# freshman97/LinTransUNet

Measured on AMD Instinct MI355X. Metric: 128^3 CT patches/sec (fwd+bwd), higher is better.
Workload: dtype bf16; 1 GPU; MaskTransUnet train step (fwd + 5-level loss + bwd), 128^3 single-channel patches, 2 per GPU, dropout 0.3, random-init weights; global_batch=2, parallelism=dp1, side_stream_concurrent=True, allreduce=none (1 rank)

## Files before the change

### lintransunet_amd/csrc/sdgrad_ring.hip

```cpp
#include "gemm_desc.h"
#include "lds_dma.h"

struct SdEnt { int c, dh, dw, dd, tap; };
template <int SD>
__host__ __device__ constexpr SdEnt sd_entry(int e) {
  int idx = 0, cls = 0;
  for (int ph = 0; ph < 2; ++ph)
    for (int pw = 0; pw < 2; ++pw)
      for (int pd = 0; pd < SD; ++pd) {
        const int nh = ph ? 2 : 1, nw = pw ? 2 : 1, nd = SD == 2 ? (pd ? 2 : 1) : 3;
        for (int i = 0; i < nh; ++i)
          for (int j = 0; j < nw; ++j)
            for (int k = 0; k < nd; ++k) {
              if (idx == e) {
                const int oh = ph ? (i == 0 ? 1 : 0) : 0, th = ph ? (i == 0 ? 0 : 2) : 1;
                const int ow = pw ? (j == 0 ? 1 : 0) : 0, tw = pw ? (j == 0 ? 0 : 2) : 1;
                const int od = SD == 2 ? (pd ? (k == 0 ? 1 : 0) : 0) : 1 - k;
                const int td = SD == 2 ? (pd ? (k == 0 ? 0 : 2) : 1) : k;
                return SdEnt{cls, oh, ow, od, (th * 3 + tw) * 3 + td};
              }
              ++idx;
            }
        ++cls;
      }
  return SdEnt{0, 0, 0, 0, -1};
}

struct SdgradArgs {
  const uint16_t* g;
  const uint16_t* w;
  uint16_t* dx;
  int B, Ho, Wo, Do, Co;
  int Hl, Wl, Dl, N;
  int tap[28];
};

template <int SD>
__global__ void __launch_bounds__(256) sdgrad_ring_bf16_kernel(const SdgradArgs a) {
  constexpr int NC = SD == 2 ? 8 : 4;
  constexpr int HH = 5, HW = 9, HD = SD == 2 ? 9 : 10;
  constexpr int NR = HH * HW * HD, HP = ((NR + 15) / 16 + 3) / 4;
  constexpr int HBUF = 4 * HP * 1024;
  constexpr int WSTAGE = 20 * 1024;
  constexpr int RING = 2 * HBUF;
  constexpr int OD0 = SD == 2 ? 0 : 1;
  extern __shared__ __attribute__((aligned(1024))) char smem[];
  const int tid = threadIdx.x, lane = tid & 63, wave = tid >> 6;
  const int li = lane & 31, lh = lane >> 5;
  const int nbh = (a.Ho + 3) / 4, nbw = (a.Wo + 7) / 8, nbd = (a.Do + 7) / 8;
  const Brick bk = split_brick(blockIdx.x, nbh, nbw, nbd);
  const int b = bk.b, h0 = bk.bh * 4, w0 = bk.bw * 8, d0 = bk.bd * 8;
  const int n_blk = blockIdx.y * 32;
  const int nchunk = a.Co / 32;
  const int total = nchunk * 3;
  const uint32_t lds0 = lds_addr(smem);
  const uint16_t* zsrc = reinterpret_cast<const uint16_t*>(ltu_zero_line) + (lane & 3) * 8;

  const int prow = lane >> 2;
  const uint16_t* hsrc[HP];
#pragma unroll
  for (int s = 0; s < HP; ++s) {
    const int hv = (wave * HP + s) * 16 + prow;
    const int hd = hv % HD, hw = (hv / HD) % HW, hh = hv / (HD * HW);
    const int h = h0 + hh, w = w0 + hw, d = d0 - OD0 + hd;
    const int lc = (lane & 3) ^ (hw & 3);
    const bool in = hv < NR && (unsigned)h < (unsigned)a.Ho && (unsigned)w < (unsigned)a.Wo && (unsigned)d < (unsigned)a.Do;
    hsrc[s] = in ? a.g + ((((long long)b * a.Ho + h) * a.Wo + w) * a.Do + d) * a.Co + lc * 8 : zsrc;
  }
  const uint16_t* wsrc[3][5];
#pragma unroll
  for (int s = 0; s < 5; ++s) {
    const int row = (wave * 5 + s) * 16 + prow;
    const int t = row >> 5, n = n_blk + (row & 31);
    const int wchunk = (lane & 3) ^ ((lane >> 4) & 3);
#pragma unroll
    for (int st = 0; st < 3; ++st) {
      const int tap = t < 9 ? a.tap[st * 9 + t] : 27;
      wsrc[st][s] = (tap < 27 && n < a.N) ? a.w + ((long long)n * 27 + tap) * a.Co + wchunk * 8 : zsrc;
    }
  }
  asm volatile("s_waitcnt vmcnt(0)" ::: "memory");

  auto issue_halo = [&](int chunk) {
    const uint32_t hb = lds0 + (chunk & 1) * HBUF + wave * HP * 1024;
#pragma unroll
    for (int s = 0; s < HP; ++s) glds16(hsrc[s] + chunk * 32, hb + s * 1024);
  };
  auto issue_w = [&](int chunk, auto ST) {
    constexpr int st = decltype(ST)::value;
    const uint32_t wb = lds0 + RING + st * WSTAGE + wave * 5 * 1024;
#pragma unroll
    for (int s = 0; s < 5; ++s) glds16(wsrc[st][s] + chunk * 32, wb + s * 1024);
  };

  const int hwl = li >> 3;
  int baseA[2][2][2];
#pragma unroll
  for (int i = 0; i < 2; ++i) {
    const int hv0 = ((wave * HW) + (i * 4 + hwl)) * HD + (li & 7);
#pragma unroll
    for (int ks = 0; ks < 2; ++ks)
#pragma unroll
      for (int dw = 0; dw < 2; ++dw) baseA[i][ks][dw] = hv0 * 64 + (((ks * 2 + lh) ^ ((hwl + dw) & 3)) << 4);
  }
  int baseW[2];
#pragma unroll
  for (int ks = 0; ks < 2; ++ks) baseW[ks] = RING + li * 64 + (((ks * 2 + lh) ^ ((li >> 2) & 3)) << 4);

  f32x16 acc[NC][2];
#pragma unroll
  for (int c = 0; c < NC; ++c)
#pragma unroll
    for (int i = 0; i < 2; ++i)
#pragma unroll
      for (int r = 0; r < 16; ++r) acc[c][i][r] = 0.f;

  issue_halo(0);
  issue_w(0, std::integral_constant<int, 0>{});
  issue_w(0, std::integral_constant<int, 1>{});
  for (int chunk = 0; chunk < nchunk; ++chunk) {
    const int hoff = (chunk & 1) * HBUF;
    int bA[2][2][2];
#pragma unroll
    for (int i = 0; i < 2; ++i)
#pragma unroll
      for (int ks = 0; ks < 2; ++ks)
#pragma unroll
        for (int dw = 0; dw < 2; ++dw) bA[i][ks][dw] = baseA[i][ks][dw] + hoff;
    static_for<0, 3>([&](auto ST) {
      constexpr int st = decltype(ST)::value;
      const int g = chunk * 3 + st;
      if (g + 1 < total) {
        if (st != 0 && chunk + 1 < nchunk) ring_sync<5 + HP>(); else ring_sync<5>();
      } else {
        ring_sync<0>();
      }
      if (g + 2 < total) {
        if constexpr (st == 0) issue_w(chunk, std::integral_constant<int, 2>{});
        else issue_w(chunk + 1, std::integral_constant<int, st - 1>{});
      }
      if (st == 0 && chunk + 1 < nchunk) issue_halo(chunk + 1);
      constexpr int NE = 9;
      auto load_frags = [&](auto TT, bf16x8 (&af)[2][2], bf16x8 (&wf)[2]) {
        constexpr int t = decltype(TT)::value;
        constexpr SdEnt en = sd_entry<SD>(st * 9 + t);
        constexpr int immA = ((en.dh * HW + en.dw) * HD + en.dd + OD0) * 64;
        constexpr int immW = st * WSTAGE + t * 2048;
#pragma unroll
        for (int i = 0; i < 2; ++i)
#pragma unroll
          for (int ks = 0; ks < 2; ++ks) af[i][ks] = *reinterpret_cast<const bf16x8*>(smem + bA[i][ks][en.dw] + immA);
#pragma unroll
        for (int ks = 0; ks < 2; ++ks) wf[ks] = *reinterpret_cast<const bf16x8*>(smem + baseW[ks] + immW);
      };
      auto mma = [&](auto TT, const bf16x8 (&af)[2][2], const bf16x8 (&wf)[2]) {
        constexpr int c = sd_entry<SD>(st * 9 + decltype(TT)::value).c;
#pragma unroll
        for (int ks = 0; ks < 2; ++ks)
#pragma unroll
          for (int i = 0; i < 2; ++i) acc[c][i] = __builtin_amdgcn_mfma_f32_32x32x16_bf16(wf[ks], af[i][ks], acc[c][i], 0, 0, 0);
      };
      bf16x8 afA[2][2], wfA[2], afB[2][2], wfB[2];
      load_frags(std::integral_constant<int, 0>{}, afA, wfA);
      static_for<0, (NE + 1) / 2>([&](auto TP) {
        constexpr int t = decltype(TP)::value * 2;
        if constexpr (t + 1 < NE) load_frags(std::integral_constant<int, t + 1>{}, afB, wfB);
        __builtin_amdgcn_sched_barrier(0);
        mma(std::integral_constant<int, t>{}, afA, wfA);
        __builtin_amdgcn_sched_barrier(0);
        if constexpr (t + 2 < NE) load_frags(std::integral_constant<int, t + 2>{}, afA, wfA);
        __builtin_amdgcn_sched_barrier(0);
        if constexpr (t + 1 < NE) mma(std::integral_constant<int, t + 1>{}, afB, wfB);
        __builtin_amdgcn_sched_barrier(0);
      });
    });
  }

  __syncthreads();
#pragma unroll
  for (int c = 0; c < NC; ++c)
#pragma unroll
    for (int i = 0; i < 2; ++i) {
      const int vox = wave * 64 + i * 32 + li;
      char* row = smem + (c * 256 + vox) * 64;
#pragma unroll
      for (int rr = 0; rr < 4; ++rr) {
        uint2 pk;
        pk.x = pack_bf16x2(acc[c][i][4 * rr + 0], acc[c][i][4 * rr + 1]);
        pk.y = pack_bf16x2(acc[c][i][4 * rr + 2], acc[c][i][4 * rr + 3]);
        *reinterpret_cast<uint2*>(row + ((rr ^ ((vox >> 1) & 3)) << 4) + lh * 8) = pk;
      }
    }
  __syncthreads();
  const int part = tid & 3;
  const bool pok = n_blk + part * 8 < a.N;
  long long vbase[4];
  int qq[4];
#pragma unroll
  for (int k = 0; k < 4; ++k) {
    const int ml = (tid >> 2) + 64 * k;
    const int qh = h0 + (ml >> 6), qw = w0 + ((ml >> 3) & 7), qd = d0 + (ml & 7);
    const bool ok = pok && qh < a.Ho && qw < a.Wo && qd < a.Do;
    vbase[k] = ((((long long)b * a.Hl + 2 * qh) * a.Wl + 2 * qw) * a.Dl + SD * qd) * a.N + n_blk + part * 8;
    qq[k] = ok ? (qh << 20) | (qw << 10) | qd : -1;
  }
#pragma unroll
  for (int c = 0; c < NC; ++c) {
    const int ph = SD == 2 ? c >> 2 : c >> 1, pw = SD == 2 ? (c >> 1) & 1 : c & 1, pd = SD == 2 ? c & 1 : 0;
    const long long coff = ((long long)(ph * a.Wl + pw) * a.Dl + pd) * a.N;
#pragma unroll
    for (int k = 0; k < 4; ++k) {
      const int ml = (tid >> 2) + 64 * k;
      const uint4 v = *reinterpret_cast<const uint4*>(smem + (c * 256 + ml) * 64 + ((part ^ ((ml >> 1) & 3)) << 4));
      const int qh = qq[k] >> 20, qw = (qq[k] >> 10) & 1023, qd = qq[k] & 1023;
      if (qq[k] >= 0 && 2 * qh + ph < a.Hl && 2 * qw + pw < a.Wl && SD * qd + pd < a.Dl)
        *reinterpret_cast<uint4*>(a.dx + vbase[k] + coff) = v;
    }
  }
}

template <int SD>
static int launch_sdgrad(const SdgradArgs& a0, hipStream_t st) {
  SdgradArgs a = a0;
  for (int e = 0; e < 27; ++e) a.tap[e] = sd_entry<SD>(e).tap;
  a.tap[27] = 27;
  constexpr int HD = SD == 2 ? 9 : 10;
  constexpr int HP = ((5 * 9 * HD + 15) / 16 + 3) / 4;
  constexpr int opnd = 2 * 4 * HP * 1024 + 3 * 20 * 1024, epi = (SD == 2 ? 8 : 4) * 256 * 64;
  constexpr int smem_bytes = opnd > epi ? opnd : epi;
  static LtuDevOnce attr_once;
  if (attr_once.first())
    ltu_dyn_lds(&sdgrad_ring_bf16_kernel<SD>, smem_bytes);
  const long long rb = (long long)a.B * ((a.Ho + 3) / 4) * ((a.Wo + 7) / 8) * ((a.Do + 7) / 8);
  if (rb >= (1LL << 31)) return 1;
  hipLaunchKernelGGL(sdgrad_ring_bf16_kernel<SD>, dim3((unsigned)rb, (a.N + 31) / 32), dim3(256), smem_bytes, st, a);
  return ltu_check_launch();
}

int launch_sdgrad_ring_bf16(const void* grad, const void* wd, void* dx, int B, int Hl, int Wl, int Dl, int N, int Co, int sd, hipStream_t st) {
  if (Co % 32 || Co > 512 || N % 8 || (sd != 1 && sd != 2)) return 1;
  SdgradArgs a;
  a.g = (const uint16_t*)grad; a.w = (const uint16_t*)wd; a.dx = (uint16_t*)dx;
  a.B = B; a.Hl = Hl; a.Wl = Wl; a.Dl = Dl; a.N = N; a.Co = Co;
  a.Ho = (Hl - 1) / 2 + 1; a.Wo = (Wl - 1) / 2 + 1; a.Do = (Dl - 1) / sd + 1;
  if (a.Ho < 1 || a.Wo < 1 || a.Do < 1 || a.Ho >= 1024 || a.Wo >= 1024 || a.Do >= 1024) return 1;
  if ((long long)N * 27 * Co >= (1LL << 31)) return 1;
  return sd == 2 ? launch_sdgrad<2>(a, st) : launch_sdgrad<1>(a, st);
}
```

### lintransunet_amd/csrc/upconv_ring.hip

```cpp
#include "gemm_desc.h"
#include "lds_dma.h"

#define UR_HROWS 640
#define UR_HBUF (UR_HROWS * 64)
#define UR_RING (2 * UR_HBUF)
#define UR_WSTAGE 16384
#define UR_SMEM (UR_RING + 4 * UR_WSTAGE)

__host__ __device__ constexpr int ur_off(int p, int a) { return p == 0 ? (a == 0 ? -1 : 0) : (a == 0 ? 0 : 1); }

struct UpRingArgs {
  const uint16_t* x;
  const uint16_t* w;
  const float* bias;
  uint16_t* y;
  int B, H, W, D, Ci, Co;
};

__global__ void __launch_bounds__(256) upconv_ring_bf16_kernel(const UpRingArgs a) {
  extern __shared__ __attribute__((aligned(1024))) char smem[];
  const int tid = threadIdx.x, lane = tid & 63, wave = tid >> 6;
  const int li = lane & 31, lh = lane >> 5;
  const int nbh = (a.H + 3) / 4, nbw = (a.W + 7) / 8, nbd = (a.D + 7) / 8;
  const Brick bk = split_brick(blockIdx.x, nbh, nbw, nbd);
  const int b = bk.b, h0 = bk.bh * 4, w0 = bk.bw * 8, d0 = bk.bd * 8;
  const int n_blk = blockIdx.y * 32;
  const int nchunk = a.Ci / 32;
  const int total = nchunk * 8;
  const uint32_t lds0 = lds_addr(smem);

  const int prow = lane >> 2;
  const uint16_t* hsrc[10];
#pragma unroll
  for (int s = 0; s < 10; ++s) {
    const int hv = (wave * 10 + s) * 16 + prow;
    const int hd = hv % 10, hw = (hv / 10) % 10, hh = hv / 100;
    const int h = h0 - 1 + hh, w = w0 - 1 + hw, d = d0 - 1 + hd;
    const int lc = (lane & 3) ^ (hw & 3);
    const bool in = hv < 600 && (unsigned)h < (unsigned)a.H && (unsigned)w < (unsigned)a.W && (unsigned)d < (unsigned)a.D;
    hsrc[s] = in ? a.x + ((((long long)b * a.H + h) * a.W + w) * a.D + d) * a.Ci + lc * 8
                 : reinterpret_cast<const uint16_t*>(ltu_zero_line) + (lane & 3) * 8;
  }
  int woff[4];
#pragma unroll
  for (int s = 0; s < 4; ++s) {
    const int row = (wave * 4 + s) * 16 + prow;
    const int t = row >> 5, n = n_blk + (row & 31);
    const int wchunk = (lane & 3) ^ ((lane >> 4) & 3);
    woff[s] = (n * 8 + t) * a.Ci + wchunk * 8;
  }
  const int wcls = a.Co * 8 * a.Ci;

  auto issue_halo = [&](int chunk) {
    const uint32_t hb = lds0 + (chunk & 1) * UR_HBUF + wave * 10 * 1024;
#pragma unroll
    for (int s = 0; s < 10; ++s) glds16(hsrc[s] + chunk * 32, hb + s * 1024);
  };
  auto issue_w = [&](int g) {
    const uint16_t* wsrc = a.w + (long long)(g & 7) * wcls + (g >> 3) * 32;
    const uint32_t wb = lds0 + UR_RING + (g & 3) * UR_WSTAGE + wave * 4 * 1024;
#pragma unroll
    for (int s = 0; s < 4; ++s) glds16(wsrc + woff[s], wb + s * 1024);
  };

  const int hwl = li >> 3;
  int baseA[2][2][3];
#pragma unroll
  for (int i = 0; i < 2; ++i) {
    const int hv0 = ((wave + 1) * 10 + (i * 4 + hwl + 1)) * 10 + (li & 7) + 1;
#pragma unroll
    for (int ks = 0; ks < 2; ++ks)
#pragma unroll
      for (int dwi = 0; dwi < 3; ++dwi) baseA[i][ks][dwi] = (hv0 - 111) * 64 + (((ks * 2 + lh) ^ ((hwl + dwi) & 3)) << 4);
  }
  int baseW[2];
#pragma unroll
  for (int ks = 0; ks < 2; ++ks) baseW[ks] = UR_RING + li * 64 + (((ks * 2 + lh) ^ ((li >> 2) & 3)) << 4);

  f32x16 acc[8][2];
#pragma unroll
  for (int c = 0; c < 8; ++c)
#pragma unroll
    for (int i = 0; i < 2; ++i)
#pragma unroll
      for (int r = 0; r < 16; ++r) acc[c][i][r] = 0.f;

  issue_halo(0);
  for (int g = 0; g < 3 && g < total; ++g) issue_w(g);
  for (int chunk = 0; chunk < nchunk; ++chunk) {
    const int hoff = (chunk & 1) * UR_HBUF;
    int bA[2][2][3];
#pragma unroll
    for (int i = 0; i < 2; ++i)
#pragma unroll
      for (int ks = 0; ks < 2; ++ks)
#pragma unroll
        for (int dwi = 0; dwi < 3; ++dwi) bA[i][ks][dwi] = baseA[i][ks][dwi] + hoff;
    static_for<0, 8>([&](auto ST) {
      constexpr int c = decltype(ST)::value;
      const int g = chunk * 8 + c;
      if (g + 2 < total) {
        constexpr bool near0 = c >= 1 && c <= 3;
        if (near0 && chunk + 1 < nchunk) ring_sync<18>(); else ring_sync<8>();
      } else {
        ring_sync<0>();
      }
      if (g + 3 < total) issue_w(g + 3);
      if (c == 0 && chunk + 1 < nchunk) issue_halo(chunk + 1);
      constexpr int ph = c >> 2, pw = (c >> 1) & 1, pd = c & 1;
      auto load_frags = [&](auto TT, bf16x8 (&af)[2][2], bf16x8 (&wf)[2]) {
        constexpr int t = decltype(TT)::value;
        constexpr int dh = ur_off(ph, t >> 2), dw = ur_off(pw, (t >> 1) & 1), dd = ur_off(pd, t & 1);
        constexpr int immA = (((dh * 10 + dw) * 10 + dd) + 111) * 64;
        constexpr int immW = (c & 3) * UR_WSTAGE + t * 2048;
#pragma unroll
        for (int i = 0; i < 2; ++i)
#pragma unroll
          for (int ks = 0; ks < 2; ++ks) af[i][ks] = *reinterpret_cast<const bf16x8*>(smem + bA[i][ks][dw + 1] + immA);
#pragma unroll
        for (int ks = 0; ks < 2; ++ks) wf[ks] = *reinterpret_cast<const bf16x8*>(smem + baseW[ks] + immW);
      };
      auto mma = [&](const bf16x8 (&af)[2][2], const bf16x8 (&wf)[2]) {
#pragma unroll
        for (int ks = 0; ks < 2; ++ks)
#pragma unroll
          for (int i = 0; i < 2; ++i) acc[c][i] = __builtin_amdgcn_mfma_f32_32x32x16_bf16(wf[ks], af[i][ks], acc[c][i], 0, 0, 0);
      };
      bf16x8 afA[2][2], wfA[2], afB[2][2], wfB[2];
      load_frags(std::integral_constant<int, 0>{}, afA, wfA);
      static_for<0, 4>([&](auto TP) {
        constexpr int t = decltype(TP)::value * 2;
        load_frags(std::integral_constant<int, t + 1>{}, afB, wfB);
        __builtin_amdgcn_sched_barrier(0);
        mma(afA, wfA);
        __builtin_amdgcn_sched_barrier(0);
        if constexpr (t + 2 < 8) load_frags(std::integral_constant<int, t + 2>{}, afA, wfA);
        __builtin_amdgcn_sched_barrier(0);
        mma(afB, wfB);
        __builtin_amdgcn_sched_barrier(0);
      });
    });
  }

  float4 bv4[4];
#pragma unroll
  for (int rr = 0; rr < 4; ++rr) {
    const int n = n_blk + 8 * rr + 4 * lh;
    bv4[rr] = a.bias != nullptr ? *reinterpret_cast<const float4*>(a.bias + n) : make_float4(0.f, 0.f, 0.f, 0.f);
  }
  __syncthreads();
#pragma unroll
  for (int c = 0; c < 8; ++c)
#pragma unroll
    for (int i = 0; i < 2; ++i) {
      const int vox = wave * 64 + i * 32 + li;
      char* row = smem + (c * 256 + vox) * 64;
#pragma unroll
      for (int rr = 0; rr < 4; ++rr) {
        uint2 pk;
        pk.x = pack_bf16x2(acc[c][i][4 * rr + 0] + bv4[rr].x, acc[c][i][4 * rr + 1] + bv4[rr].y);
        pk.y = pack_bf16x2(acc[c][i][4 * rr + 2] + bv4[rr].z, acc[c][i][4 * rr + 3] + bv4[rr].w);
        *reinterpret_cast<uint2*>(row + ((rr ^ ((vox >> 1) & 3)) << 4) + lh * 8) = pk;
      }
    }
  __syncthreads();
  const int part = tid & 3;
  const int Hh = 2 * a.H, Wh = 2 * a.W, Dh = 2 * a.D;
  long long vbase[4];
#pragma unroll
  for (int k = 0; k < 4; ++k) {
    const int ml = (tid >> 2) + 64 * k;
    const int qh = h0 + (ml >> 6), qw = w0 + ((ml >> 3) & 7), qd = d0 + (ml & 7);
    const bool ok = qh < a.H && qw < a.W && qd < a.D;
    vbase[k] = ok ? ((((long long)b * Hh + 2 * qh) * Wh + 2 * qw) * Dh + 2 * qd) * a.Co + n_blk + part * 8 : -1;
  }
#pragma unroll
  for (int c = 0; c < 8; ++c) {
    const long long coff = ((long long)((c >> 2) * Wh + ((c >> 1) & 1)) * Dh + (c & 1)) * a.Co;
#pragma unroll
    for (int k = 0; k < 4; ++k) {
      const int ml = (tid >> 2) + 64 * k;
      const uint4 v = *reinterpret_cast<const uint4*>(smem + (c * 256 + ml) * 64 + ((part ^ ((ml >> 1) & 3)) << 4));
      if (vbase[k] >= 0) *reinterpret_cast<uint4*>(a.y + vbase[k] + coff) = v;
    }
  }
}

int launch_upconv_ring_bf16(const void* x, const void* wsub_f, const float* bias, void* y, int B, int H, int W, int D, int Ci, int Co,
                            hipStream_t st) {
  if (Ci % 32 || Co % 32 || Ci > 512 || H < 2 || W < 4 || D < 2) return 1;
  const long long rb = (long long)B * ((H + 3) / 4) * ((W + 7) / 8) * ((D + 7) / 8);
  if (rb >= (1LL << 31) || (long long)8 * Co * 8 * Ci >= (1LL << 31)) return 1;
  static LtuDevOnce attr_once;
  if (attr_once.first())
    ltu_dyn_lds(&upconv_ring_bf16_kernel, UR_SMEM);
  UpRingArgs a;
  a.x = (const uint16_t*)x; a.w = (const uint16_t*)wsub_f; a.bias = bias; a.y = (uint16_t*)y;
  a.B = B; a.H = H; a.W = W; a.D = D; a.Ci = Ci; a.Co = Co;
  hipLaunchKernelGGL(upconv_ring_bf16_kernel, dim3((unsigned)rb, Co / 32), dim3(256), UR_SMEM, st, a);
  return ltu_check_launch();
}
```

### lintransunet_amd/csrc/updgrad_ring.hip

```cpp
#include "gemm_desc.h"
#include "lds_dma.h"

#define UG_HP 7
#define UG_HBUF (4 * UG_HP * 1024)
#define UG_RING (2 * UG_HBUF)
#define UG_WSTAGE 16384
#define UG_SMEM (UG_RING + 4 * UG_WSTAGE)

struct UpDgradArgs {
  const uint16_t* g;
  const uint16_t* w;
  uint16_t* dx;
  int B, H, W, D, Ci, Co;
};

template <int TN>
__global__ void __launch_bounds__(256) updgrad_ring_bf16_kernel(const UpDgradArgs a) {
  constexpr int BN = 32 * TN, WSLOT = BN * 64, WST = 2 * WSLOT;
  extern __shared__ __attribute__((aligned(1024))) char smem[];
  const int tid = threadIdx.x, lane = tid & 63, wave = tid >> 6;
  const int li = lane & 31, lh = lane >> 5;
  const int nbh = (a.H + 3) / 4, nbw = (a.W + 7) / 8, nbd = (a.D + 7) / 8;
  const Brick bk = split_brick(blockIdx.x, nbh, nbw, nbd);
  const int b = bk.b, h0 = bk.bh * 4, w0 = bk.bw * 8, d0 = bk.bd * 8;
  const int n_blk = blockIdx.y * BN;
  const int nchunk = a.Co / 32;
  const int total = nchunk * 32;
  const int Hf = 2 * a.H, Wf = 2 * a.W, Df = 2 * a.D;
  const uint32_t lds0 = lds_addr(smem);
  const char* zsrc = reinterpret_cast<const char*>(ltu_zero_line) + (lane & 3) * 16;
  const int prow = lane >> 2;

  long long hoffs[UG_HP];
  int hfc[UG_HP];
#pragma unroll
  for (int s = 0; s < UG_HP; ++s) {
    const int hv = (wave * UG_HP + s) * 16 + prow;
    const int hd = hv % 9, hw = (hv / 9) % 9, hh = hv / 81;
    const int fh = 2 * (h0 + hh), fw = 2 * (w0 + hw), fd = 2 * (d0 + hd);
    const int lc = (lane & 3) ^ (hw & 3);
    hoffs[s] = hv < 405 ? ((((long long)b * Hf + fh) * Wf + fw) * Df + fd) * a.Co + lc * 8 : -1;
    hfc[s] = fh | (fw << 10) | (fd << 20);
  }
  auto issue_halo = [&](int chunk, auto PP) {
    constexpr int p = decltype(PP)::value, ph = p >> 2, pw = (p >> 1) & 1, pd = p & 1;
    const uint32_t hb = lds0 + (p & 1) * UG_HBUF + wave * UG_HP * 1024;
    const long long delta = (((long long)ph * Wf + pw) * Df + pd) * a.Co - chunk * 32;
#pragma unroll
    for (int s = 0; s < UG_HP; ++s) {
      const int fh = (hfc[s] & 1023) - ph, fw = ((hfc[s] >> 10) & 1023) - pw, fd = (hfc[s] >> 20) - pd;
      const bool in = hoffs[s] >= 0 && (unsigned)fh < (unsigned)Hf && (unsigned)fw < (unsigned)Wf && (unsigned)fd < (unsigned)Df;
      const char* src = in ? reinterpret_cast<const char*>(a.g + (hoffs[s] - delta)) : zsrc;
      glds16(src, hb + s * 1024);
    }
  };
  int woff[TN];
#pragma unroll
  for (int s = 0; s < TN; ++s) {
    const int pp = wave * TN + s, sl2 = pp / (BN / 16), n = n_blk + (pp % (BN / 16)) * 16 + prow;
    const int wchunk = (lane & 3) ^ ((lane >> 4) & 3);
    woff[s] = (n * 64 + sl2) * a.Co + wchunk * 8;
  }
  auto issue_w = [&](int g) {
    const int chunk = g >> 5, e0 = (g & 31) * 2;
    const uint16_t* wsrc = a.w + e0 * a.Co + chunk * 32;
    const uint32_t wb = lds0 + UG_RING + (g & 3) * UG_WSTAGE + wave * TN * 1024;
#pragma unroll
    for (int s = 0; s < TN; ++s) glds16(wsrc + woff[s], wb + s * 1024);
  };

  const int hwl = li >> 3;
  int baseA[2][2][2];
#pragma unroll
  for (int i = 0; i < 2; ++i) {
    const int hv0 = (wave * 9 + (i * 4 + hwl)) * 9 + (li & 7);
#pragma unroll
    for (int ks = 0; ks < 2; ++ks)
#pragma unroll
      for (int dw = 0; dw < 2; ++dw) baseA[i][ks][dw] = hv0 * 64 + (((ks * 2 + lh) ^ ((hwl + dw) & 3)) << 4);
  }
  int baseW[2];
#pragma unroll
  for (int ks = 0; ks < 2; ++ks) baseW[ks] = UG_RING + li * 64 + (((ks * 2 + lh) ^ ((li >> 2) & 3)) << 4);

  f32x16 acc[2][TN];
#pragma unroll
  for (int i = 0; i < 2; ++i)
#pragma unroll
    for (int j = 0; j < TN; ++j)
#pragma unroll
      for (int r = 0; r < 16; ++r) acc[i][j][r] = 0.f;

  issue_halo(0, std::integral_constant<int, 0>{});
  for (int g = 0; g < 3 && g < total; ++g) issue_w(g);
  for (int chunk = 0; chunk < nchunk; ++chunk) {
    static_for<0, 32>([&](auto ST) {
      constexpr int st = decltype(ST)::value, p = st >> 2, q = st & 3;
      const int g = chunk * 32 + st;
      const bool halo_next = p < 7 || chunk + 1 < nchunk;
      if (g + 2 < total) {
        if (q != 0 && halo_next) ring_sync<2 * TN + UG_HP>(); else ring_sync<2 * TN>();
      } else {
        ring_sync<0>();
      }
      if (g + 3 < total) issue_w(g + 3);
      if constexpr (q == 0) {
        if (halo_next) {
          if constexpr (p < 7) issue_halo(chunk, std::integral_constant<int, p + 1>{});
          else issue_halo(chunk + 1, std::integral_constant<int, 0>{});
        }
      }
      auto load_frags = [&](auto TT, bf16x8 (&af)[2][2], bf16x8 (&wf)[TN][2]) {
        constexpr int t = decltype(TT)::value, sl = 2 * q + t;
        constexpr int dh = 1 - (sl >> 2), dw = 1 - ((sl >> 1) & 1), dd = 1 - (sl & 1);
        constexpr int immA = ((dh * 9 + dw) * 9 + dd) * 64 + (p & 1) * UG_HBUF;
        constexpr int immW = q * UG_WSTAGE + t * WSLOT;
#pragma unroll
        for (int i = 0; i < 2; ++i)
#pragma unroll
          for (int ks = 0; ks < 2; ++ks) af[i][ks] = *reinterpret_cast<const bf16x8*>(smem + baseA[i][ks][dw] + immA);
#pragma unroll
        for (int j = 0; j < TN; ++j)
#pragma unroll
          for (int ks = 0; ks < 2; ++ks) wf[j][ks] = *reinterpret_cast<const bf16x8*>(smem + baseW[ks] + immW + j * 2048);
      };
      auto mma = [&](const bf16x8 (&af)[2][2], const bf16x8 (&wf)[TN][2]) {
#pragma unroll
        for (int ks = 0; ks < 2; ++ks)
#pragma unroll
          for (int j = 0; j < TN; ++j)
#pragma unroll
            for (int i = 0; i < 2; ++i) acc[i][j] = __builtin_amdgcn_mfma_f32_32x32x16_bf16(wf[j][ks], af[i][ks], acc[i][j], 0, 0, 0);
      };
      bf16x8 afA[2][2], wfA[TN][2], afB[2][2], wfB[TN][2];
      load_frags(std::integral_constant<int, 0>{}, afA, wfA);
      load_frags(std::integral_constant<int, 1>{}, afB, wfB);
      __builtin_amdgcn_sched_barrier(0);
      mma(afA, wfA);
      __builtin_amdgcn_sched_barrier(0);
      mma(afB, wfB);
      __builtin_amdgcn_sched_barrier(0);
    });
  }

  constexpr int PARTS = BN / 8, RB = 2 * BN;
  __syncthreads();
#pragma unroll
  for (int i = 0; i < 2; ++i) {
    const int row = wave * 64 + i * 32 + li;
#pragma unroll
    for (int j = 0; j < TN; ++j)
#pragma unroll
      for (int rr = 0; rr < 4; ++rr) {
        uint2 pk;
        pk.x = pack_bf16x2(acc[i][j][4 * rr + 0], acc[i][j][4 * rr + 1]);
        pk.y = pack_bf16x2(acc[i][j][4 * rr + 2], acc[i][j][4 * rr + 3]);
        *reinterpret_cast<uint2*>(smem + row * RB + (((j * 4 + rr) ^ (row & (PARTS - 1))) << 4) + lh * 8) = pk;
      }
  }
  __syncthreads();
#pragma unroll 4
  for (int it = 0; it < PARTS; ++it) {
    const int idx = it * 256 + tid, part = idx & (PARTS - 1), row = idx / PARTS;
    const int qh = h0 + (row >> 6), qw = w0 + ((row >> 3) & 7), qd = d0 + (row & 7);
    const uint4 v = *reinterpret_cast<const uint4*>(smem + row * RB + ((part ^ (row & (PARTS - 1))) << 4));
    if (qh < a.H && qw < a.W && qd < a.D)
      *reinterpret_cast<uint4*>(a.dx + ((((long long)b * a.H + qh) * a.W + qw) * a.D + qd) * a.Ci + n_blk + part * 8) = v;
  }
}

int launch_updgrad_ring_bf16(const void* grad, const void* wsub_d, void* dx, int B, int H, int W, int D, int Ci, int Co, hipStream_t st) {
  if (Ci % 128 || Co % 32 || Co > 512 || H < 2 || W < 4 || D < 2 || 2 * H >= 1024 || 2 * W >= 1024 || 2 * D >= 1024) return 1;
  const long long rb = (long long)B * ((H + 3) / 4) * ((W + 7) / 8) * ((D + 7) / 8);
  if (rb >= (1LL << 31) || (long long)Ci * 64 * Co >= (1LL << 31)) return 1;
  static LtuDevOnce attr_once;
  if (attr_once.first()) {
    ltu_dyn_lds(&updgrad_ring_bf16_kernel<4>, UG_SMEM);
    ltu_dyn_lds(&updgrad_ring_bf16_kernel<2>, UG_SMEM);
  }
  UpDgradArgs a;
  a.g = (const uint16_t*)grad; a.w = (const uint16_t*)wsub_d; a.dx = (uint16_t*)dx;
  a.B = B; a.H = H; a.W = W; a.D = D; a.Ci = Ci; a.Co = Co;
  if (rb * (Ci / 128) < ltu_knob_pos("LTU_UPDGRAD_WIDE_MIN", 160))
    hipLaunchKernelGGL(updgrad_ring_bf16_kernel<2>, dim3((unsigned)rb, Ci / 64), dim3(256), UG_SMEM, st, a);
  else
    hipLaunchKernelGGL(updgrad_ring_bf16_kernel<4>, dim3((unsigned)rb, Ci / 128), dim3(256), UG_SMEM, st, a);
  return ltu_check_launch();
}
```

Measured before the change: 163.1 patches/s.

## Interleave ring DMA issues between MFMAs and prefetch next stage fragments across syncs

In the sdgrad, upconv and updgrad ring kernels, the global-to-LDS weight and halo loads are split into single pieces and issued between individual MFMA instructions instead of in one burst at the start of each stage. The first fragment load of the next stage is moved ahead of the current stage's last MFMAs, so the ring sync and the LDS reads overlap with math. The halo base offset is now advanced in place rather than recomputed per chunk, and a nchunk>=1 assumption is added with matching launch guards. This is meant to hide barrier and LDS latency and smooth memory-queue pressure, at the cost of more complex schedules and a new ring_sync_all primitive whose wait-count correctness is critical.

```diff
diff --git a/lintransunet_amd/csrc/sdgrad_ring.hip b/lintransunet_amd/csrc/sdgrad_ring.hip
--- a/lintransunet_amd/csrc/sdgrad_ring.hip
+++ b/lintransunet_amd/csrc/sdgrad_ring.hip
@@ -52,7 +52,7 @@
   const int b = bk.b, h0 = bk.bh * 4, w0 = bk.bw * 8, d0 = bk.bd * 8;
   const int n_blk = blockIdx.y * 32;
   const int nchunk = a.Co / 32;
-  const int total = nchunk * 3;
+  __builtin_assume(nchunk >= 1);
   const uint32_t lds0 = lds_addr(smem);
   const uint16_t* zsrc = reinterpret_cast<const uint16_t*>(ltu_zero_line) + (lane & 3) * 8;
 
@@ -81,17 +81,16 @@
   }
   asm volatile("s_waitcnt vmcnt(0)" ::: "memory");
 
-  auto issue_halo = [&](int chunk) {
-    const uint32_t hb = lds0 + (chunk & 1) * HBUF + wave * HP * 1024;
-#pragma unroll
-    for (int s = 0; s < HP; ++s) glds16(hsrc[s] + chunk * 32, hb + s * 1024);
-  };
-  auto issue_w = [&](int chunk, auto ST) {
-    constexpr int st = decltype(ST)::value;
-    const uint32_t wb = lds0 + RING + st * WSTAGE + wave * 5 * 1024;
-#pragma unroll
-    for (int s = 0; s < 5; ++s) glds16(wsrc[st][s] + chunk * 32, wb + s * 1024);
-  };
+  auto issue_halo_piece = [&](int chunk, auto SS) {
+    constexpr int s = decltype(SS)::value;
+    glds16(hsrc[s] + chunk * 32, lds0 + (chunk & 1) * HBUF + (wave * HP + s) * 1024);
+  };
+  auto issue_w_piece = [&](int chunk, auto ST, auto SS) {
+    constexpr int st = decltype(ST)::value, s = decltype(SS)::value;
+    glds16(wsrc[st][s] + chunk * 32, lds0 + RING + st * WSTAGE + (wave * 5 + s) * 1024);
+  };
+  auto issue_halo = [&](int chunk) { static_for<0, HP>([&](auto SS) { issue_halo_piece(chunk, SS); }); };
+  auto issue_w = [&](int chunk, auto ST) { static_for<0, 5>([&](auto SS) { issue_w_piece(chunk, ST, SS); }); };
 
   const int hwl = li >> 3;
   int baseA[2][2][2];
@@ -114,66 +113,82 @@
     for (int i = 0; i < 2; ++i)
 #pragma unroll
       for (int r = 0; r < 16; ++r) acc[c][i][r] = 0.f;
+
+  auto load_frags = [&](auto ST, auto TT, bf16x8 (&af)[2][2], bf16x8 (&wf)[2]) {
+    constexpr int st = decltype(ST)::value, t = decltype(TT)::value;
+    constexpr SdEnt en = sd_entry<SD>(st * 9 + t);
+    constexpr int immA = ((en.dh * HW + en.dw) * HD + en.dd + OD0) * 64;
+    constexpr int immW = st * WSTAGE + t * 2048;
+#pragma unroll
+    for (int i = 0; i < 2; ++i)
+#pragma unroll
+      for (int ks = 0; ks < 2; ++ks) af[i][ks] = *reinterpret_cast<const bf16x8*>(smem + baseA[i][ks][en.dw] + immA);
+#pragma unroll
+    for (int ks = 0; ks < 2; ++ks) wf[ks] = *reinterpret_cast<const bf16x8*>(smem + baseW[ks] + immW);
+  };
+  auto stage_sync = [&](auto ST, bool more) {
+    constexpr int st = decltype(ST)::value;
+    if (st <= 1 || more) {
+      if (st != 0 && more) ring_sync_all<5 + HP>(); else ring_sync_all<5>();
+    } else {
+      ring_sync_all<0>();
+    }
+  };
+
+  bf16x8 af[2][2][2], wf[2][2];
+  auto run_chunk = [&](auto PAR, int chunk) {
+    const bool more = chunk + 1 < nchunk;
+    static_for<0, 3>([&](auto ST) {
+      constexpr int st = decltype(ST)::value;
+      auto piece = [&](auto PP) {
+        constexpr int P = decltype(PP)::value;
+        if constexpr (st == 0) {
+          if constexpr (P < 5) issue_w_piece(chunk, std::integral_constant<int, 2>{}, PP);
+          else if constexpr (P < 5 + HP) { if (more) issue_halo_piece(chunk + 1, std::integral_constant<int, P - 5>{}); }
+        } else if constexpr (P % 3 == 1 && P < 15) {
+          if (more) issue_w_piece(chunk + 1, std::integral_constant<int, st - 1>{}, std::integral_constant<int, P / 3>{});
+        }
+      };
+      static_for<0, 9>([&](auto TT) {
+        constexpr int t = decltype(TT)::value, cur = (decltype(PAR)::value + st * 9 + t) & 1, nxt = cur ^ 1;
+        if constexpr (t + 1 < 9) {
+          load_frags(ST, std::integral_constant<int, t + 1>{}, af[nxt], wf[nxt]);
+        } else if (st < 2 || more) {
+          constexpr int sn = (st + 1) % 3;
+          stage_sync(std::integral_constant<int, sn>{}, st == 2 ? chunk + 2 < nchunk : more);
+          if constexpr (st == 2) {
+            const int hstep = (chunk & 1) ? -HBUF : HBUF;
+#pragma unroll
+            for (int i = 0; i < 2; ++i)
+#pragma unroll
+              for (int ks = 0; ks < 2; ++ks)
+#pragma unroll
+                for (int dw = 0; dw < 2; ++dw) baseA[i][ks][dw] += hstep;
+          }
+          load_frags(std::integral_constant<int, sn>{}, std::integral_constant<int, 0>{}, af[nxt], wf[nxt]);
+        }
+        __builtin_amdgcn_sched_barrier(0);
+        constexpr int c = sd_entry<SD>(st * 9 + t).c;
+        static_for<0, 2>([&](auto KS) {
+          constexpr int ks = decltype(KS)::value;
+#pragma unroll
+          for (int i = 0; i < 2; ++i) acc[c][i] = __builtin_amdgcn_mfma_f32_32x32x16_bf16(wf[cur][ks], af[cur][i][ks], acc[c][i], 0, 0, 0);
+          __builtin_amdgcn_sched_barrier(0);
+          piece(std::integral_constant<int, t * 2 + ks>{});
+          __builtin_amdgcn_sched_barrier(0);
+        });
+      });
+    });
+  };
 
   issue_halo(0);
   issue_w(0, std::integral_constant<int, 0>{});
   issue_w(0, std::integral_constant<int, 1>{});
-  for (int chunk = 0; chunk < nchunk; ++chunk) {
-    const int hoff = (chunk & 1) * HBUF;
-    int bA[2][2][2];
-#pragma unroll
-    for (int i = 0; i < 2; ++i)
-#pragma unroll
-      for (int ks = 0; ks < 2; ++ks)
-#pragma unroll
-        for (int dw = 0; dw < 2; ++dw) bA[i][ks][dw] = baseA[i][ks][dw] + hoff;
-    static_for<0, 3>([&](auto ST) {
-      constexpr int st = decltype(ST)::value;
-      const int g = chunk * 3 + st;
-      if (g + 1 < total) {
-        if (st != 0 && chunk + 1 < nchunk) ring_sync<5 + HP>(); else ring_sync<5>();
-      } else {
-        ring_sync<0>();
-      }
-      if (g + 2 < total) {
-        if constexpr (st == 0) issue_w(chunk, std::integral_constant<int, 2>{});
-        else issue_w(chunk + 1, std::integral_constant<int, st - 1>{});
-      }
-      if (st == 0 && chunk + 1 < nchunk) issue_halo(chunk + 1);
-      constexpr int NE = 9;
-      auto load_frags = [&](auto TT, bf16x8 (&af)[2][2], bf16x8 (&wf)[2]) {
-        constexpr int t = decltype(TT)::value;
-        constexpr SdEnt en = sd_entry<SD>(st * 9 + t);
-        constexpr int immA = ((en.dh * HW + en.dw) * HD + en.dd + OD0) * 64;
-        constexpr int immW = st * WSTAGE + t * 2048;
-#pragma unroll
-        for (int i = 0; i < 2; ++i)
-#pragma unroll
-          for (int ks = 0; ks < 2; ++ks) af[i][ks] = *reinterpret_cast<const bf16x8*>(smem + bA[i][ks][en.dw] + immA);
-#pragma unroll
-        for (int ks = 0; ks < 2; ++ks) wf[ks] = *reinterpret_cast<const bf16x8*>(smem + baseW[ks] + immW);
-      };
-      auto mma = [&](auto TT, const bf16x8 (&af)[2][2], const bf16x8 (&wf)[2]) {
-        constexpr int c = sd_entry<SD>(st * 9 + decltype(TT)::value).c;
-#pragma unroll
-        for (int ks = 0; ks < 2; ++ks)
-#pragma unroll
-          for (int i = 0; i < 2; ++i) acc[c][i] = __builtin_amdgcn_mfma_f32_32x32x16_bf16(wf[ks], af[i][ks], acc[c][i], 0, 0, 0);
-      };
-      bf16x8 afA[2][2], wfA[2], afB[2][2], wfB[2];
-      load_frags(std::integral_constant<int, 0>{}, afA, wfA);
-      static_for<0, (NE + 1) / 2>([&](auto TP) {
-        constexpr int t = decltype(TP)::value * 2;
-        if constexpr (t + 1 < NE) load_frags(std::integral_constant<int, t + 1>{}, afB, wfB);
-        __builtin_amdgcn_sched_barrier(0);
-        mma(std::integral_constant<int, t>{}, afA, wfA);
-        __builtin_amdgcn_sched_barrier(0);
-        if constexpr (t + 2 < NE) load_frags(std::integral_constant<int, t + 2>{}, afA, wfA);
-        __builtin_amdgcn_sched_barrier(0);
-        if constexpr (t + 1 < NE) mma(std::integral_constant<int, t + 1>{}, afB, wfB);
-        __builtin_amdgcn_sched_barrier(0);
-      });
-    });
+  stage_sync(std::integral_constant<int, 0>{}, nchunk > 1);
+  load_frags(std::integral_constant<int, 0>{}, std::integral_constant<int, 0>{}, af[0], wf[0]);
+  for (int chunk = 0; chunk < nchunk; chunk += 2) {
+    run_chunk(std::integral_constant<int, 0>{}, chunk);
+    if (chunk + 1 < nchunk) run_chunk(std::integral_constant<int, 1>{}, chunk + 1);
   }
 
   __syncthreads();
@@ -238,7 +253,7 @@
 }
 
 int launch_sdgrad_ring_bf16(const void* grad, const void* wd, void* dx, int B, int Hl, int Wl, int Dl, int N, int Co, int sd, hipStream_t st) {
-  if (Co % 32 || Co > 512 || N % 8 || (sd != 1 && sd != 2)) return 1;
+  if (Co < 32 || Co % 32 || Co > 512 || N % 8 || (sd != 1 && sd != 2)) return 1;
   SdgradArgs a;
   a.g = (const uint16_t*)grad; a.w = (const uint16_t*)wd; a.dx = (uint16_t*)dx;
   a.B = B; a.Hl = Hl; a.Wl = Wl; a.Dl = Dl; a.N = N; a.Co = Co;
diff --git a/lintransunet_amd/csrc/upconv_ring.hip b/lintransunet_amd/csrc/upconv_ring.hip
--- a/lintransunet_amd/csrc/upconv_ring.hip
+++ b/lintransunet_amd/csrc/upconv_ring.hip
@@ -26,6 +26,7 @@
   const int b = bk.b, h0 = bk.bh * 4, w0 = bk.bw * 8, d0 = bk.bd * 8;
   const int n_blk = blockIdx.y * 32;
   const int nchunk = a.Ci / 32;
+  __builtin_assume(nchunk >= 1);
   const int total = nchunk * 8;
   const uint32_t lds0 = lds_addr(smem);
 
@@ -51,17 +52,17 @@
   }
   const int wcls = a.Co * 8 * a.Ci;
 
-  auto issue_halo = [&](int chunk) {
-    const uint32_t hb = lds0 + (chunk & 1) * UR_HBUF + wave * 10 * 1024;
-#pragma unroll
-    for (int s = 0; s < 10; ++s) glds16(hsrc[s] + chunk * 32, hb + s * 1024);
-  };
-  auto issue_w = [&](int g) {
+  auto issue_halo_piece = [&](int chunk, auto SS) {
+    constexpr int s = decltype(SS)::value;
+    glds16(hsrc[s] + chunk * 32, lds0 + (chunk & 1) * UR_HBUF + (wave * 10 + s) * 1024);
+  };
+  auto issue_w_piece = [&](int g, auto SS) {
+    constexpr int s = decltype(SS)::value;
     const uint16_t* wsrc = a.w + (long long)(g & 7) * wcls + (g >> 3) * 32;
-    const uint32_t wb = lds0 + UR_RING + (g & 3) * UR_WSTAGE + wave * 4 * 1024;
-#pragma unroll
-    for (int s = 0; s < 4; ++s) glds16(wsrc + woff[s], wb + s * 1024);
-  };
+    glds16(wsrc + woff[s], lds0 + UR_RING + (g & 3) * UR_WSTAGE + (wave * 4 + s) * 1024);
+  };
+  auto issue_halo = [&](int chunk) { static_for<0, 10>([&](auto SS) { issue_halo_piece(chunk, SS); }); };
+  auto issue_w = [&](int g) { static_for<0, 4>([&](auto SS) { issue_w_piece(g, SS); }); };
 
   const int hwl = li >> 3;
   int baseA[2][2][3];
@@ -85,59 +86,81 @@
 #pragma unroll
       for (int r = 0; r < 16; ++r) acc[c][i][r] = 0.f;
 
+  auto load_frags = [&](auto CC, auto TT, bf16x8 (&af)[2][2], bf16x8 (&wf)[2]) {
+    constexpr int c = decltype(CC)::value, t = decltype(TT)::value;
+    constexpr int ph = c >> 2, pw = (c >> 1) & 1, pd = c & 1;
+    constexpr int dh = ur_off(ph, t >> 2), dw = ur_off(pw, (t >> 1) & 1), dd = ur_off(pd, t & 1);
+    constexpr int immA = (((dh * 10 + dw) * 10 + dd) + 111) * 64;
+    constexpr int immW = (c & 3) * UR_WSTAGE + t * 2048;
+#pragma unroll
+    for (int i = 0; i < 2; ++i)
+#pragma unroll
+      for (int ks = 0; ks < 2; ++ks) af[i][ks] = *reinterpret_cast<const bf16x8*>(smem + baseA[i][ks][dw + 1] + immA);
+#pragma unroll
+    for (int ks = 0; ks < 2; ++ks) wf[ks] = *reinterpret_cast<const bf16x8*>(smem + baseW[ks] + immW);
+  };
+  auto stage_sync = [&](auto CC, bool more) {
+    constexpr int c = decltype(CC)::value;
+    if (c <= 5 || more) {
+      if (c >= 1 && c <= 3 && more) ring_sync_all<18>(); else ring_sync_all<8>();
+    } else {
+      ring_sync_all<0>();
+    }
+  };
+
+  bf16x8 afA[2][2], wfA[2], afB[2][2], wfB[2];
   issue_halo(0);
   for (int g = 0; g < 3 && g < total; ++g) issue_w(g);
+  stage_sync(std::integral_constant<int, 0>{}, nchunk > 1);
+  load_frags(std::integral_constant<int, 0>{}, std::integral_constant<int, 0>{}, afA, wfA);
   for (int chunk = 0; chunk < nchunk; ++chunk) {
-    const int hoff = (chunk & 1) * UR_HBUF;
-    int bA[2][2][3];
-#pragma unroll
-    for (int i = 0; i < 2; ++i)
-#pragma unroll
-      for (int ks = 0; ks < 2; ++ks)
-#pragma unroll
-        for (int dwi = 0; dwi < 3; ++dwi) bA[i][ks][dwi] = baseA[i][ks][dwi] + hoff;
+    const bool more = chunk + 1 < nchunk;
     static_for<0, 8>([&](auto ST) {
       constexpr int c = decltype(ST)::value;
       const int g = chunk * 8 + c;
-      if (g + 2 < total) {
-        constexpr bool near0 = c >= 1 && c <= 3;
-        if (near0 && chunk + 1 < nchunk) ring_sync<18>(); else ring_sync<8>();
-      } else {
-        ring_sync<0>();
-      }
-      if (g + 3 < total) issue_w(g + 3);
-      if (c == 0 && chunk + 1 < nchunk) issue_halo(chunk + 1);
-      constexpr int ph = c >> 2, pw = (c >> 1) & 1, pd = c & 1;
-      auto load_frags = [&](auto TT, bf16x8 (&af)[2][2], bf16x8 (&wf)[2]) {
-        constexpr int t = decltype(TT)::value;
-        constexpr int dh = ur_off(ph, t >> 2), dw = ur_off(pw, (t >> 1) & 1), dd = ur_off(pd, t & 1);
-        constexpr int immA = (((dh * 10 + dw) * 10 + dd) + 111) * 64;
-        constexpr int immW = (c & 3) * UR_WSTAGE + t * 2048;
-#pragma unroll
-        for (int i = 0; i < 2; ++i)
-#pragma unroll
-          for (int ks = 0; ks < 2; ++ks) af[i][ks] = *reinterpret_cast<const bf16x8*>(smem + bA[i][ks][dw + 1] + immA);
-#pragma unroll
-        for (int ks = 0; ks < 2; ++ks) wf[ks] = *reinterpret_cast<const bf16x8*>(smem + baseW[ks] + immW);
+      const bool w3 = c <= 4 || more;
+      auto piece = [&](auto PP) {
+        constexpr int P = decltype(PP)::value;
+        if constexpr (c == 0) {
+          if constexpr (P < 4) issue_w_piece(g + 3, PP);
+          else if constexpr (P < 14) { if (more) issue_halo_piece(chunk + 1, std::integral_constant<int, P - 4>{}); }
+        } else if constexpr (P % 3 == 1 && P < 12) {
+          if (w3) issue_w_piece(g + 3, std::integral_constant<int, P / 3>{});
+        }
       };
-      auto mma = [&](const bf16x8 (&af)[2][2], const bf16x8 (&wf)[2]) {
-#pragma unroll
-        for (int ks = 0; ks < 2; ++ks)
+      auto mma = [&](auto TT, const bf16x8 (&af)[2][2], const bf16x8 (&wf)[2]) {
+        static_for<0, 2>([&](auto KS) {
+          constexpr int ks = decltype(KS)::value;
 #pragma unroll
           for (int i = 0; i < 2; ++i) acc[c][i] = __builtin_amdgcn_mfma_f32_32x32x16_bf16(wf[ks], af[i][ks], acc[c][i], 0, 0, 0);
+          __builtin_amdgcn_sched_barrier(0);
+          piece(std::integral_constant<int, decltype(TT)::value * 2 + ks>{});
+          __builtin_amdgcn_sched_barrier(0);
+        });
       };
-      bf16x8 afA[2][2], wfA[2], afB[2][2], wfB[2];
-      load_frags(std::integral_constant<int, 0>{}, afA, wfA);
       static_for<0, 4>([&](auto TP) {
         constexpr int t = decltype(TP)::value * 2;
-        load_frags(std::integral_constant<int, t + 1>{}, afB, wfB);
+        load_frags(ST, std::integral_constant<int, t + 1>{}, afB, wfB);
         __builtin_amdgcn_sched_barrier(0);
-        mma(afA, wfA);
+        mma(std::integral_constant<int, t>{}, afA, wfA);
+        if constexpr (t + 2 < 8) {
+          load_frags(ST, std::integral_constant<int, t + 2>{}, afA, wfA);
+        } else if (c < 7 || more) {
+          constexpr int cn = (c + 1) & 7;
+          stage_sync(std::integral_constant<int, cn>{}, c == 7 ? chunk + 2 < nchunk : more);
+          if constexpr (c == 7) {
+            const int hstep = (chunk & 1) ? -UR_HBUF : UR_HBUF;
+#pragma unroll
+            for (int i = 0; i < 2; ++i)
+#pragma unroll
+              for (int ks = 0; ks < 2; ++ks)
+#pragma unroll
+                for (int dwi = 0; dwi < 3; ++dwi) baseA[i][ks][dwi] += hstep;
+          }
+          load_frags(std::integral_constant<int, cn>{}, std::integral_constant<int, 0>{}, afA, wfA);
+        }
         __builtin_amdgcn_sched_barrier(0);
-        if constexpr (t + 2 < 8) load_frags(std::integral_constant<int, t + 2>{}, afA, wfA);
-        __builtin_amdgcn_sched_barrier(0);
-        mma(afB, wfB);
-        __builtin_amdgcn_sched_barrier(0);
+        mma(std::integral_constant<int, t + 1>{}, afB, wfB);
       });
     });
   }
@@ -188,7 +211,7 @@
 
 int launch_upconv_ring_bf16(const void* x, const void* wsub_f, const float* bias, void* y, int B, int H, int W, int D, int Ci, int Co,
                             hipStream_t st) {
-  if (Ci % 32 || Co % 32 || Ci > 512 || H < 2 || W < 4 || D < 2) return 1;
+  if (Ci < 32 || Ci % 32 || Co % 32 || Ci > 512 || H < 2 || W < 4 || D < 2) return 1;
   const long long rb = (long long)B * ((H + 3) / 4) * ((W + 7) / 8) * ((D + 7) / 8);
   if (rb >= (1LL << 31) || (long long)8 * Co * 8 * Ci >= (1LL << 31)) return 1;
   static LtuDevOnce attr_once;
diff --git a/lintransunet_amd/csrc/updgrad_ring.hip b/lintransunet_amd/csrc/updgrad_ring.hip
--- a/lintransunet_amd/csrc/updgrad_ring.hip
+++ b/lintransunet_amd/csrc/updgrad_ring.hip
@@ -16,7 +16,7 @@
 
 template <int TN>
 __global__ void __launch_bounds__(256) updgrad_ring_bf16_kernel(const UpDgradArgs a) {
-  constexpr int BN = 32 * TN, WSLOT = BN * 64, WST = 2 * WSLOT;
+  constexpr int BN = 32 * TN, WSLOT = BN * 64;
   extern __shared__ __attribute__((aligned(1024))) char smem[];
   const int tid = threadIdx.x, lane = tid & 63, wave = tid >> 6;
   const int li = lane & 31, lh = lane >> 5;
@@ -42,18 +42,15 @@
     hoffs[s] = hv < 405 ? ((((long long)b * Hf + fh) * Wf + fw) * Df + fd) * a.Co + lc * 8 : -1;
     hfc[s] = fh | (fw << 10) | (fd << 20);
   }
-  auto issue_halo = [&](int chunk, auto PP) {
-    constexpr int p = decltype(PP)::value, ph = p >> 2, pw = (p >> 1) & 1, pd = p & 1;
-    const uint32_t hb = lds0 + (p & 1) * UG_HBUF + wave * UG_HP * 1024;
+  auto issue_halo_piece = [&](int chunk, auto PP, auto SS) {
+    constexpr int p = decltype(PP)::value, ph = p >> 2, pw = (p >> 1) & 1, pd = p & 1, s = decltype(SS)::value;
     const long long delta = (((long long)ph * Wf + pw) * Df + pd) * a.Co - chunk * 32;
-#pragma unroll
-    for (int s = 0; s < UG_HP; ++s) {
-      const int fh = (hfc[s] & 1023) - ph, fw = ((hfc[s] >> 10) & 1023) - pw, fd = (hfc[s] >> 20) - pd;
-      const bool in = hoffs[s] >= 0 && (unsigned)fh < (unsigned)Hf && (unsigned)fw < (unsigned)Wf && (unsigned)fd < (unsigned)Df;
-      const char* src = in ? reinterpret_cast<const char*>(a.g + (hoffs[s] - delta)) : zsrc;
-      glds16(src, hb + s * 1024);
-    }
-  };
+    const int fh = (hfc[s] & 1023) - ph, fw = ((hfc[s] >> 10) & 1023) - pw, fd = (hfc[s] >> 20) - pd;
+    const bool in = hoffs[s] >= 0 && (unsigned)fh < (unsigned)Hf && (unsigned)fw < (unsigned)Wf && (unsigned)fd < (unsigned)Df;
+    const char* src = in ? reinterpret_cast<const char*>(a.g + (hoffs[s] - delta)) : zsrc;
+    glds16(src, lds0 + (p & 1) * UG_HBUF + (wave * UG_HP + s) * 1024);
+  };
+  auto issue_halo = [&](int chunk, auto PP) { static_for<0, UG_HP>([&](auto SS) { issue_halo_piece(chunk, PP, SS); }); };
   int woff[TN];
 #pragma unroll
   for (int s = 0; s < TN; ++s) {
@@ -61,13 +58,13 @@
     const int wchunk = (lane & 3) ^ ((lane >> 4) & 3);
     woff[s] = (n * 64 + sl2) * a.Co + wchunk * 8;
   }
-  auto issue_w = [&](int g) {
+  auto issue_w_piece = [&](int g, auto SS) {
+    constexpr int s = decltype(SS)::value;
     const int chunk = g >> 5, e0 = (g & 31) * 2;
     const uint16_t* wsrc = a.w + e0 * a.Co + chunk * 32;
-    const uint32_t wb = lds0 + UG_RING + (g & 3) * UG_WSTAGE + wave * TN * 1024;
-#pragma unroll
-    for (int s = 0; s < TN; ++s) glds16(wsrc + woff[s], wb + s * 1024);
-  };
+    glds16(wsrc + woff[s], lds0 + UG_RING + (g & 3) * UG_WSTAGE + (wave * TN + s) * 1024);
+  };
+  auto issue_w = [&](int g) { static_for<0, TN>([&](auto SS) { issue_w_piece(g, SS); }); };
 
   const int hwl = li >> 3;
   int baseA[2][2][2];
@@ -91,54 +88,80 @@
 #pragma unroll
       for (int r = 0; r < 16; ++r) acc[i][j][r] = 0.f;
 
+  constexpr int NM = 4 * TN;
+  auto load_frags = [&](auto ST, auto TT, bf16x8 (&af)[2][2], bf16x8 (&wf)[TN][2]) {
+    constexpr int st = decltype(ST)::value, p = st >> 2, q = st & 3;
+    constexpr int t = decltype(TT)::value, sl = 2 * q + t;
+    constexpr int dh = 1 - (sl >> 2), dw = 1 - ((sl >> 1) & 1), dd = 1 - (sl & 1);
+    constexpr int immA = ((dh * 9 + dw) * 9 + dd) * 64 + (p & 1) * UG_HBUF;
+    constexpr int immW = q * UG_WSTAGE + t * WSLOT;
+#pragma unroll
+    for (int i = 0; i < 2; ++i)
+#pragma unroll
+      for (int ks = 0; ks < 2; ++ks) af[i][ks] = *reinterpret_cast<const bf16x8*>(smem + baseA[i][ks][dw] + immA);
+#pragma unroll
+    for (int j = 0; j < TN; ++j)
+#pragma unroll
+      for (int ks = 0; ks < 2; ++ks) wf[j][ks] = *reinterpret_cast<const bf16x8*>(smem + baseW[ks] + immW + j * 2048);
+  };
+  auto stage_sync = [&](auto ST, bool more) {
+    constexpr int st = decltype(ST)::value, p = st >> 2, q = st & 3;
+    if (st <= 29 || more) {
+      if (q != 0 && (p < 7 || more)) ring_sync_all<2 * TN + UG_HP>(); else ring_sync_all<2 * TN>();
+    } else {
+      ring_sync_all<0>();
+    }
+  };
+
+  bf16x8 afA[2][2], wfA[TN][2], afB[2][2], wfB[TN][2];
   issue_halo(0, std::integral_constant<int, 0>{});
   for (int g = 0; g < 3 && g < total; ++g) issue_w(g);
+  stage_sync(std::integral_constant<int, 0>{}, nchunk > 1);
+  load_frags(std::integral_constant<int, 0>{}, std::integral_constant<int, 0>{}, afA, wfA);
   for (int chunk = 0; chunk < nchunk; ++chunk) {
+    const bool more = chunk + 1 < nchunk;
     static_for<0, 32>([&](auto ST) {
       constexpr int st = decltype(ST)::value, p = st >> 2, q = st & 3;
       const int g = chunk * 32 + st;
-      const bool halo_next = p < 7 || chunk + 1 < nchunk;
-      if (g + 2 < total) {
-        if (q != 0 && halo_next) ring_sync<2 * TN + UG_HP>(); else ring_sync<2 * TN>();
-      } else {
-        ring_sync<0>();
+      const bool w3 = st <= 28 || more;
+      const bool halo_next = p < 7 || more;
+      auto halo_piece = [&](auto SS) {
+        if constexpr (p < 7) issue_halo_piece(chunk, std::integral_constant<int, p + 1>{}, SS);
+        else issue_halo_piece(chunk + 1, std::integral_constant<int, 0>{}, SS);
+      };
+      auto piece = [&](auto MM) {
+        constexpr int M = decltype(MM)::value;
+        if constexpr (q == 0) {
+          if constexpr (M < TN) { if (w3) issue_w_piece(g + 3, MM); }
+          else if constexpr (M < TN + UG_HP) { if (halo_next) halo_piece(std::integral_constant<int, M - TN>{}); }
+          if constexpr (M == NM - 1 && NM < TN + UG_HP) {
+            if (halo_next) static_for<NM - TN, UG_HP>([&](auto SS) { halo_piece(SS); });
+          }
+        } else if constexpr (M % 4 == 1) {
+          if (w3) issue_w_piece(g + 3, std::integral_constant<int, M / 4>{});
+        }
+      };
+      load_frags(ST, std::integral_constant<int, 1>{}, afB, wfB);
+      __builtin_amdgcn_sched_barrier(0);
+      static_for<0, NM>([&](auto MM) {
+        constexpr int M = decltype(MM)::value, ks = M / (2 * TN), j = (M / 2) % TN, i = M & 1;
+        acc[i][j] = __builtin_amdgcn_mfma_f32_32x32x16_bf16(wfA[j][ks], afA[i][ks], acc[i][j], 0, 0, 0);
+        __builtin_amdgcn_sched_barrier(0);
+        piece(MM);
+        __builtin_amdgcn_sched_barrier(0);
+      });
+      if (st < 31 || more) {
+        constexpr int sn = (st + 1) & 31;
+        stage_sync(std::integral_constant<int, sn>{}, st == 31 ? chunk + 2 < nchunk : more);
+        load_frags(std::integral_constant<int, sn>{}, std::integral_constant<int, 0>{}, afA, wfA);
       }
-      if (g + 3 < total) issue_w(g + 3);
-      if constexpr (q == 0) {
-        if (halo_next) {
-          if constexpr (p < 7) issue_halo(chunk, std::integral_constant<int, p + 1>{});
-          else issue_halo(chunk + 1, std::integral_constant<int, 0>{});
-        }
-      }
-      auto load_frags = [&](auto TT, bf16x8 (&af)[2][2], bf16x8 (&wf)[TN][2]) {
-        constexpr int t = decltype(TT)::value, sl = 2 * q + t;
-        constexpr int dh = 1 - (sl >> 2), dw = 1 - ((sl >> 1) & 1), dd = 1 - (sl & 1);
-        constexpr int immA = ((dh * 9 + dw) * 9 + dd) * 64 + (p & 1) * UG_HBUF;
-        constexpr int immW = q * UG_WSTAGE + t * WSLOT;
-#pragma unroll
-        for (int i = 0; i < 2; ++i)
-#pragma unroll
-          for (int ks = 0; ks < 2; ++ks) af[i][ks] = *reinterpret_cast<const bf16x8*>(smem + baseA[i][ks][dw] + immA);
+      __builtin_amdgcn_sched_barrier(0);
+#pragma unroll
+      for (int ks = 0; ks < 2; ++ks)
 #pragma unroll
         for (int j = 0; j < TN; ++j)
 #pragma unroll
-          for (int ks = 0; ks < 2; ++ks) wf[j][ks] = *reinterpret_cast<const bf16x8*>(smem + baseW[ks] + immW + j * 2048);
-      };
-      auto mma = [&](const bf16x8 (&af)[2][2], const bf16x8 (&wf)[TN][2]) {
-#pragma unroll
-        for (int ks = 0; ks < 2; ++ks)
-#pragma unroll
-          for (int j = 0; j < TN; ++j)
-#pragma unroll
-            for (int i = 0; i < 2; ++i) acc[i][j] = __builtin_amdgcn_mfma_f32_32x32x16_bf16(wf[j][ks], af[i][ks], acc[i][j], 0, 0, 0);
-      };
-      bf16x8 afA[2][2], wfA[TN][2], afB[2][2], wfB[TN][2];
-      load_frags(std::integral_constant<int, 0>{}, afA, wfA);
-      load_frags(std::integral_constant<int, 1>{}, afB, wfB);
-      __builtin_amdgcn_sched_barrier(0);
-      mma(afA, wfA);
-      __builtin_amdgcn_sched_barrier(0);
-      mma(afB, wfB);
+          for (int i = 0; i < 2; ++i) acc[i][j] = __builtin_amdgcn_mfma_f32_32x32x16_bf16(wfB[j][ks], afB[i][ks], acc[i][j], 0, 0, 0);
       __builtin_amdgcn_sched_barrier(0);
     });
   }
```

Result: no change. 163.9 patches/s, median of 6 (+0.5%).
